# azuxmioy/Render-In-Between

Hardware: AMD Instinct MI355X
Metric: rendered frames/sec at 512x512 (generator forward + blend, device-resident) (higher is better)
Workload: dtype f32

## Files before the change

include/rib.h:

```cpp
#ifndef RIB_H
#define RIB_H

#include <stddef.h>
#include <stdint.h>

#ifdef __cplusplus
extern "C" {
#endif

typedef struct rib_handle rib_handle;

typedef enum {
  RIB_OK = 0,
  RIB_ERR_INVALID = -1,
  RIB_ERR_UNSUPPORTED = -2,
  RIB_ERR_STATE = -3,
  RIB_ERR_MISSING = -4,
  RIB_ERR_HIP = -5,
  RIB_ERR_WORKSPACE = -6
} rib_status;

typedef struct {
  int32_t label_nc;
  int32_t image_nc;
// ... 104 lines not shown
int rib_time_op(rib_handle* h, int B, int H, int W, const char* op_name, const float* label,
                const float* img_fake, const float* img_prev, float* img, float* mask, void* workspace,
                size_t workspace_bytes, int iters, void* hip_stream, double* usec);

int rib_set_graph_replay(rib_handle* h, int enable);
int rib_graph_stats(rib_handle* h, int64_t* captures, int64_t* replays);

int rib_set_plan_batch(rib_handle* h, int n);
int rib_get_plan_batch(const rib_handle* h);

const char* rib_build_info(void);

int rib_debug_conv_weight(rib_handle* h, const char* conv_name, float* w_oihw, float* bias);
int rib_debug_spade_weight(rib_handle* h, const char* conv_name, float* w_2c_by_cond, float* bias_2c);
int rib_debug_launch_info(rib_handle* h, int B, int H, int W, int idx, char* buf, size_t buflen);

#ifdef __cplusplus
}
#endif
#endif
```

render-in-between_amd/_native.py:

```python
from __future__ import annotations

import ctypes as C
import os

_HERE = os.path.dirname(os.path.abspath(__file__))
LIB_PATH = os.environ.get("RIB_LIBRARY") or os.path.join(_HERE, "csrc", "librib.so")

KC_NAMES = ("igemm", "spade", "stats", "pool", "eltwise", "pack", "conv_aux")


class RibConfig(C.Structure):
    _fields_ = [(n, C.c_int32) for n in (
        "label_nc", "image_nc", "num_filters", "max_num_filters", "num_layers", "num_down_img",
        "emb_filters", "emb_max_filters", "emb_down", "mask_filters", "mask_max_filters",
        "mask_down", "mask_res_blocks")]


class RibError(RuntimeError):
    def __init__(self, code, msg):
        super().__init__("rib error %d: %s" % (code, msg))
        self.code = code


_lib = None
# ... 47 lines not shown
    "rib_read_tap": (C.c_int, [C.c_void_p, C.c_int, C.c_int, C.c_int, C.c_int, C.c_void_p,
                               C.c_void_p, C.c_void_p]),
    "rib_profile_begin": (C.c_int, [C.c_void_p]),
    "rib_profile_begin_kernels": (C.c_int, [C.c_void_p]),
    "rib_profile_collect": (C.c_int, [C.c_void_p, C.POINTER(C.c_int64), C.POINTER(C.c_double)]),
    "rib_forward_flops": (C.c_int, [C.c_void_p, C.c_int, C.c_int, C.c_int, C.POINTER(C.c_double)]),
    "rib_num_launches": (C.c_int, [C.c_void_p, C.c_int, C.c_int, C.c_int]),
    "rib_num_variants": (C.c_int, []),
    "rib_variant_info": (C.c_int, [C.c_int, C.POINTER(C.c_int)]),
    "rib_set_choice": (C.c_int, [C.c_void_p, C.c_int, C.c_int, C.c_int, C.c_char_p, C.c_int, C.c_int]),
    "rib_time_op": (C.c_int, [C.c_void_p, C.c_int, C.c_int, C.c_int, C.c_char_p] + [C.c_void_p] * 6
                    + [C.c_size_t, C.c_int, C.c_void_p, C.POINTER(C.c_double)]),
    "rib_debug_conv_weight": (C.c_int, [C.c_void_p, C.c_char_p, C.c_void_p, C.c_void_p]),
    "rib_debug_spade_weight": (C.c_int, [C.c_void_p, C.c_char_p, C.c_void_p, C.c_void_p]),
    "rib_debug_launch_info": (C.c_int, [C.c_void_p, C.c_int, C.c_int, C.c_int, C.c_int, C.c_char_p, C.c_size_t]),
    "rib_build_info": (C.c_char_p, []),
    "rib_set_graph_replay": (C.c_int, [C.c_void_p, C.c_int]),
    "rib_graph_stats": (C.c_int, [C.c_void_p, C.POINTER(C.c_int64), C.POINTER(C.c_int64)]),
    "rib_set_plan_batch": (C.c_int, [C.c_void_p, C.c_int]),
    "rib_get_plan_batch": (C.c_int, [C.c_void_p]),
}


def lib():
    global _lib
    if _lib is None:
        if not os.path.exists(LIB_PATH):
            raise RuntimeError(
                "native library %s is missing: build it with "
                "`python render-in-between_amd/csrc/build.py` (there is no CPU fallback)" % LIB_PATH)
# ... 22 lines not shown
```

render-in-between_amd/csrc/kernels.hip.h:

```cpp
#pragma once
#include "igemm.hip.h"

namespace rib {

struct GemmDmaParams {
  const float* A; const float* B; float* C;
  int M, N, K, lda, ldc;
  size_t sA, sB, sC;
  int modB;
  int K2; unsigned long long kmask;
};

typedef uint32_t u32x4 __attribute__((ext_vector_type(4)));
__device__ __forceinline__ void split3_bf16(const float4 p, const float4 q, bf16x8& hi, bf16x8& mid, bf16x8& lo) {
  const float x[8] = {p.x, p.y, p.z, p.w, q.x, q.y, q.z, q.w};
  u32x4 h, m, l;
#pragma unroll
  for (int i = 0; i < 4; ++i) {
    const uint32_t u0 = __float_as_uint(x[2 * i]), u1 = __float_as_uint(x[2 * i + 1]);
    h[i] = __builtin_amdgcn_perm(u1, u0, 0x07060302u);
    const float r0 = x[2 * i] - __uint_as_float(u0 & 0xffff0000u), r1 = x[2 * i + 1] - __uint_as_float(u1 & 0xffff0000u);
    const uint32_t v0 = __float_as_uint(r0), v1 = __float_as_uint(r1);
    m[i] = __builtin_amdgcn_perm(v1, v0, 0x07060302u);
    const float s0 = r0 - __uint_as_float(v0 & 0xffff0000u), s1 = r1 - __uint_as_float(v1 & 0xffff0000u);
    l[i] = __builtin_amdgcn_perm(__float_as_uint(s1), __float_as_uint(s0), 0x07060302u);
  }
// ... 1 lines not shown
}

template <int WM, int WN, int NF, int ST = ST_F32, int X3 = 0>
__global__ __launch_bounds__(256) void k_gemm_dma(const GemmDmaParams p) {
  static_assert(WM * WN == 4, "4 waves per workgroup");
  static_assert(X3 == 0 || ST == ST_F32, "split products: fp32 storage");
  constexpr int BM = 32 * WM, BN = 32 * NF * WN, BK = 32;
  constexpr int EPW = ST == ST_F32 ? 1 : 2;
  constexpr int STAGE = (BM + BN) * BK;
  constexpr int NFILL = (BM + BN) / 32;
  __shared__ __attribute__((aligned(16))) float smem[2 * STAGE];
  const int tid = threadIdx.x, lane = tid & 63, li = lane & 31, lh = lane >> 5;
  const int wave = __builtin_amdgcn_readfirstlane(tid >> 6);
  const int wm = wave / WN, wn = wave % WN;
  const int m0 = blockIdx.x * BM, n0 = blockIdx.y * BN;
  const int z = blockIdx.z;
  const float* A = p.A + (size_t)z * p.sA / EPW;
  const float* B = p.B + (size_t)(p.modB ? z % p.modB : 0) * p.sB / EPW;
  f32x16 acc[NF];
  f32x16 acc_s[X3 == 2 ? NF : 1];
#pragma unroll
  for (int nf = 0; nf < NF; ++nf)
#pragma unroll
    for (int r = 0; r < 16; ++r) { acc[nf][r] = 0.f; if constexpr (X3 == 2) acc_s[nf][r] = 0.f; }
  const int ldb = (p.K + p.K2) / EPW;
  const int nch = (p.K + (p.K2 && ((p.kmask >> (z % p.modB)) & 1ull) ? p.K2 : 0)) / (BK * EPW);
  typedef __attribute__((address_space(3))) void lds_void;
  const uint32_t lds0 = (uint32_t)(size_t)(lds_void*)smem;
  const float* src[NFILL];
#pragma unroll
  for (int j = 0; j < NFILL; ++j) {
    const int trow = wave * 8 + 32 * j + (lane >> 3);
    const bool isA = 32 * j < BM;
    const int row = isA ? trow : trow - BM;
    const int ls = (lane & 7) ^ ((row >> 1) & 7);
    src[j] = isA ? A + (size_t)min(m0 + row, p.M - 1) * (p.lda / EPW) + ls * 4 : B + (size_t)min(n0 + row, p.N - 1) * ldb + ls * 4;
  }
  auto fill = [&](int st, int kc) {
#pragma unroll
    for (int j = 0; j < NFILL; ++j) {
      const uint32_t dst = lds0 + (uint32_t)(st * STAGE + (wave * 8 + 32 * j) * BK) * 4u;
// ... 46 lines not shown
#pragma unroll
      for (int nf = 0; nf < NF; ++nf) {
        if constexpr (ST == ST_F32) {
          acc[nf] = __builtin_amdgcn_mfma_f32_32x32x2f32(a.x, b[nf].x, acc[nf], 0, 0, 0);
          acc[nf] = __builtin_amdgcn_mfma_f32_32x32x2f32(a.y, b[nf].y, acc[nf], 0, 0, 0);
          acc[nf] = __builtin_amdgcn_mfma_f32_32x32x2f32(a.z, b[nf].z, acc[nf], 0, 0, 0);
          acc[nf] = __builtin_amdgcn_mfma_f32_32x32x2f32(a.w, b[nf].w, acc[nf], 0, 0, 0);
        } else if constexpr (ST == ST_F16) {
          acc[nf] = __builtin_amdgcn_mfma_f32_32x32x16_f16(*reinterpret_cast<const f16x8*>(&a), *reinterpret_cast<const f16x8*>(&b[nf]), acc[nf], 0, 0, 0);
        } else {
          acc[nf] = __builtin_amdgcn_mfma_f32_32x32x16_bf16(*reinterpret_cast<const bf16x8*>(&a), *reinterpret_cast<const bf16x8*>(&b[nf]), acc[nf], 0, 0, 0);
        }
      }
    }
  }
  float* C = p.C + (size_t)z * p.sC;
#pragma unroll
  for (int nf = 0; nf < NF; ++nf) {
    const int col = n0 + (wn * NF + nf) * 32 + li;
#pragma unroll
    for (int r = 0; r < 16; ++r) {
      const int row = m0 + wm * 32 + (r & 3) + 8 * (r >> 2) + 4 * lh;
      float v = acc[nf][r];
      if constexpr (X3 == 2) v += acc_s[nf][r];
      if (row < p.M && col < p.N) C[(size_t)row * p.ldc + col] = v;
    }
  }
}

struct FinalizeParams {
  const double* part;
// ... 340 lines not shown
  if constexpr (MODE2 >= 0) {
    const int n1 = p.nslices - p.nslices2;
    if (slice >= n1) { wino_in_slice<MODE2, true>(wino_second(p), slice - n1, ub, red, s_sc, s_sh); return; }
  }
  wino_in_slice<MODE, false>(p, slice, ub, red, s_sc, s_sh);
}

struct WinoOutParams {
  const float* m; int tilesY, tilesX, CoutPad;
  const float* bias;
  float* y; int yC, yoff, Cout, Hout, Wout;
  int act;
  const float* res; int resC;
  double* stat_part;
  int nslices, ublocks;
};

__device__ __forceinline__ void wino_out_partials(double (*red)[256][4], const double s1[4], const double s2[4], double* stat_part,
                                                  int n, int ublocks, int ub, int slice, int CoutPad) {
#pragma unroll
  for (int e = 0; e < 4; ++e) { red[0][threadIdx.x][e] = s1[e]; red[1][threadIdx.x][e] = s2[e]; }
  __syncthreads();
  if (threadIdx.x < 64) {
    const int c = slice * 64 + threadIdx.x;
    if (c < CoutPad) {
      const int g = threadIdx.x >> 2, e = threadIdx.x & 3;
      double a1 = 0.0, a2 = 0.0;
#pragma unroll
      for (int s = 0; s < 16; ++s) { a1 += red[0][s * 16 + g][e]; a2 += red[1][s * 16 + g][e]; }
      double* dst = stat_part + (((size_t)n * ublocks + ub) * 2) * CoutPad;
      dst[c] = a1;
      dst[CoutPad + c] = a2;
    }
  }
}

__global__ __launch_bounds__(256) void k_wino_out(const WinoOutParams p) {
  __shared__ __attribute__((aligned(16))) double red[2][256][4];
  const int c4n = p.CoutPad / 4;
  const int slice = blockIdx.x % p.nslices, ub = blockIdx.x / p.nslices;
  const int c4 = slice * 16 + (threadIdx.x & 15);
  const int n = blockIdx.y;
  const int ntiles = p.tilesY * p.tilesX;
  double s1[4] = {0.0, 0.0, 0.0, 0.0}, s2[4] = {0.0, 0.0, 0.0, 0.0};
  if (c4 < c4n) {
    const float4 bv = *reinterpret_cast<const float4*>(p.bias + c4 * 4);
    const size_t plane = (size_t)ntiles * p.CoutPad;
    for (int u = ub * 16 + (threadIdx.x >> 4); u < ntiles * 2; u += p.ublocks * 16) {
      const int r = u & 1, tile = u >> 1;
      const float* mb = p.m + (size_t)n * 16 * plane + (size_t)tile * p.CoutPad + c4 * 4;
      float4 mm[3][4];
#pragma unroll
      for (int a = 0; a < 3; ++a)
#pragma unroll
        for (int q = 0; q < 4; ++q) mm[a][q] = *reinterpret_cast<const float4*>(mb + (size_t)((r + a) * 4 + q) * plane);
      const float sg = r ? -1.f : 1.f;
      float4 uu[4];
#pragma unroll
      for (int q = 0; q < 4; ++q)
        uu[q] = make_float4(mm[0][q].x + sg * (mm[1][q].x + mm[2][q].x), mm[0][q].y + sg * (mm[1][q].y + mm[2][q].y),
                            mm[0][q].z + sg * (mm[1][q].z + mm[2][q].z), mm[0][q].w + sg * (mm[1][q].w + mm[2][q].w));
      float4 yv[2];
      yv[0] = RIB_F4_ADD(RIB_F4_ADD(uu[0], uu[1]), uu[2]);
      yv[1] = RIB_F4_SUB(RIB_F4_SUB(uu[1], uu[2]), uu[3]);
      const int ty = tile / p.tilesX, tx = tile % p.tilesX;
      const int oy = 2 * ty + r;
      float rr[2][4];
#pragma unroll
      for (int q = 0; q < 2; ++q) {
        const int cy = min(oy, p.Hout - 1), cx = min(2 * tx + q, p.Wout - 1);
// ... 112 lines not shown
  }
}

template <int MODE, int MODE2 = -1>
__global__ __launch_bounds__(256) void k_wino4_in(const WinoInParams p) {
  __shared__ double red[4 * 64 * 2];
  __shared__ float s_sc[64], s_sh[64];
  const int slice = blockIdx.x % p.nslices, ub = blockIdx.x / p.nslices;
  if constexpr (MODE2 >= 0) {
    const int n1 = p.nslices - p.nslices2;
    if (slice >= n1) { wino4_in_slice<MODE2, true>(wino_second(p), slice - n1, ub, red, s_sc, s_sh); return; }
  }
  wino4_in_slice<MODE, false>(p, slice, ub, red, s_sc, s_sh);
}

__global__ __launch_bounds__(256) void k_wino4_out(const WinoOutParams p) {
  __shared__ __attribute__((aligned(16))) double red[2][256][4];
  const int c4n = p.CoutPad / 4;
  const int slice = blockIdx.x % p.nslices, ub = blockIdx.x / p.nslices;
  const int c4 = slice * 16 + (threadIdx.x & 15);
  const int n = blockIdx.y;
  const int ntiles = p.tilesY * p.tilesX;
  double s1[4] = {0.0, 0.0, 0.0, 0.0}, s2[4] = {0.0, 0.0, 0.0, 0.0};
  if (c4 < c4n) {
    const float4 bv = *reinterpret_cast<const float4*>(p.bias + c4 * 4);
    const size_t plane = (size_t)ntiles * p.CoutPad;
    for (int unit = ub * 16 + (threadIdx.x >> 4); unit < ntiles * 4; unit += p.ublocks * 16) {
      const int tile = unit >> 2, r = unit & 3;
      const float* mb = p.m + (size_t)n * 36 * plane + (size_t)tile * p.CoutPad + c4 * 4;
      float4 u[6];
#pragma unroll
      for (int q = 0; q < 6; ++q) u[q] = make_float4(0.f, 0.f, 0.f, 0.f);
      const int ax = r == 0 ? 0 : 5;
      const float cx_ = (r == 0 || r == 3) ? 1.f : 0.f;
      float4 mm[5][6];
#pragma unroll
      for (int k = 0; k < 5; ++k)
#pragma unroll
        for (int q = 0; q < 6; ++q) mm[k][q] = *reinterpret_cast<const float4*>(mb + (size_t)((k < 4 ? k + 1 : ax) * 6 + q) * plane);
#pragma unroll
      for (int k = 0; k < 5; ++k) {
        const float coef = k < 4 ? kWino4AT[r][k + 1] : cx_;
#pragma unroll
        for (int q = 0; q < 6; ++q) u[q] = f4_fma(coef, mm[k][q], u[q]);
      }
      const float4 s12 = RIB_F4_ADD(u[1], u[2]);
      const float4 d12 = RIB_F4_SUB(u[1], u[2]);
      const float4 s34 = RIB_F4_ADD(u[3], u[4]);
      const float4 d34 = RIB_F4_SUB(u[3], u[4]);
      float4 yv[4];
      yv[0] = make_float4(u[0].x + s12.x + s34.x, u[0].y + s12.y + s34.y, u[0].z + s12.z + s34.z, u[0].w + s12.w + s34.w);
      yv[1] = f4_fma(3.f / 4, d12, f4_scale(3.f / 2, d34));
      yv[2] = f4_fma(9.f / 16, s12, f4_scale(9.f / 4, s34));
      yv[3] = f4_fma(27.f / 64, d12, f4_fma(27.f / 8, d34, u[5]));
// ... 653 lines not shown
```

render-in-between_amd/csrc/rib.hip:

```cpp
#include "kernels.hip.h"
#include "rib_host.h"
#include <hip/hip_ext.h>

#include <algorithm>
#include <array>
#include <climits>
#include <cmath>
#include <cstdio>
#include <cstdlib>
#include <cstring>
#include <map>
#include <memory>
#include <string>
#include <variant>
#include <vector>


#include "variants.hip.h"
#define RIB_V(sec, ...) RIB_I_V(RIB_F_EXTERN, __VA_ARGS__)
#define RIB_VK(sec, ...) RIB_I_VK(RIB_F_EXTERN, __VA_ARGS__)
#define RIB_VT(sec, ...) RIB_I_VT(RIB_F_EXTERN, __VA_ARGS__)
#define RIB_VTK(sec, ...) RIB_I_VTK(RIB_F_EXTERN, __VA_ARGS__)
#define RIB_V9(sec, ...) RIB_I_V9(RIB_F_EXTERN, __VA_ARGS__)
#define RIB_VU4(sec, ...) RIB_I_VU4(RIB_F_EXTERN, __VA_ARGS__)
// ... 786 lines not shown
struct FusionPolicy {
  bool consumer_stats = !getenv("RIB_NO_CONSUMER_STATS");
  bool head_conv = !getenv("RIB_NO_HEADCONV");
  bool small_conv = !getenv("RIB_NO_SMALLCONV");
  long wino_max_px = getenv("RIB_WINO_MAX_PX") ? atol(getenv("RIB_WINO_MAX_PX")) : 16384;
  int wino_force = getenv("RIB_WINO_M") ? atoi(getenv("RIB_WINO_M")) : 0;
  bool split_k = !getenv("RIB_NO_SPLITK");
  bool n16 = !getenv("RIB_NO_N16");
  int lowc_tw = getenv("RIB_LOWC_TW") ? (atoi(getenv("RIB_LOWC_TW")) == 16 ? 16 : 32) : 0;
  long cond_gemm_max_px = getenv("RIB_COND_GEMM_MAX_PX") ? atol(getenv("RIB_COND_GEMM_MAX_PX")) : 4096;
  bool unfused_spade = !getenv("RIB_NO_UNFUSED_SPADE");
  bool lazy_sources = !getenv("RIB_NO_LAZY");
  bool fuse_shortcut = !getenv("RIB_NO_FUSE_SHORTCUT");
  bool wino_shortcut = !getenv("RIB_NO_WINO_SHORTCUT");
  int wino_shortcut_m = getenv("RIB_WINO_SHORTCUT_M") ? atoi(getenv("RIB_WINO_SHORTCUT_M")) : 0;
  bool ws_reuse = !getenv("RIB_NO_WS_REUSE");
  static bool pair_mask_encoders() { return !getenv("RIB_NO_PAIR"); }
};

struct Builder {
  rib_handle* h;
  Plan* P;
  int B;
  const FusionPolicy pol;
  size_t ws = 0;
  std::string error;
  bool mark_label = false;
  bool pair_mask = false;
  bool defer_stats = true;
  void materialize(const Norm& n, const std::string& consumer = std::string()) {
// ... 107 lines not shown
  bool runs_wino(const ConvArgs& a, int Hout, int Wout, const std::string& opname = std::string()) const {
    const ConvDef& c = *a.cd;
    return h->prec() == PREC_F32 && (a.aux ? c.wino_s_ok : c.wino_ok) && !a.ups && !a.res_ups && !a.pair && !a.in.virt && a.y_nchw.sp == PS_NULL &&
           a.y_user.sp == PS_NULL && (long)Hout * Wout <= pol.wino_max_px && Hout >= 2 && Wout >= 2 &&
           (!a.aux || (!a.res && shortcut_wino_m(c, *a.aux, opname, Hout, Wout) != 0));
  }
  int default_wino_m(int Hout, int Wout) const { return (long)TB_() * ((Hout + 3) / 4) * ((Wout + 3) / 4) >= 256 ? 4 : 2; }
  int shortcut_wino_m(const ConvDef& c, const ConvDef& s, const std::string& opname, int Hout, int Wout) const {
    if (!pol.wino_shortcut || !pol.fuse_shortcut || opname.empty() || !c.fb_off || s.ks != 1 || s.coutp != c.coutp || s.cinp % 32 != 0 || c.cinp % 32 != 0) return 0;
    if (!pick_gemm_dma(h->prec(), 16, 64, c.coutp, c.cinp)) return 0;
    if (pol.wino_shortcut_m == 2 || pol.wino_shortcut_m == 4) return pol.wino_shortcut_m;
    const int d = default_wino_m(Hout, Wout);
    for (int m : {d, 6 - d})
      if (h->choices.count(fmt("%d,%d,%d|%s%s", TB_(), P->H, P->W, opname.c_str(), m == 2 ? ".wino" : ".wino4"))) return m;
    return 0;
  }
  bool would_wino(const ConvDef& cd, int H, int W) const { ConvArgs t; t.cd = &cd; return runs_wino(t, H, W); }

  bool conv(const ConvArgs& a, const std::string& opname) {
    const ConvDef& c = *a.cd;
    const int Hout = a.ups ? a.in.H * 2 : (c.stride == 2 ? a.in.H / 2 : a.in.H);
    const int Wout = a.ups ? a.in.W * 2 : (c.stride == 2 ? a.in.W / 2 : a.in.W);
    if (a.in.virt) return conv_lowc(a, opname);
    const int nB = a.pair ? 2 * B : B;
    if (a.pair) {
      const ConvDef& d = *a.pair;
      if (d.cinp != c.cinp || d.coutp != c.coutp || d.cout != c.cout || d.ks != c.ks || d.stride != c.stride || d.ups_in || c.ups_in || a.ups || a.res || a.aux ||
          a.y_nchw.sp != PS_NULL || a.y_user.sp != PS_NULL || a.y_none || !a.want_stats || c.in_affine != d.in_affine || d.w_off <= c.w_off || d.b_off <= c.b_off ||
          (c.in_affine && (d.g_off <= c.g_off || d.g_off - c.g_off != d.be_off - c.be_off)) || (h->mc16() && d.w16_off <= c.w16_off)) {
        error = opname + ": the two convolutions of a paired launch must have the same shape"; return false;
// ... 157 lines not shown
  }

  bool conv_wino(const ConvArgs& a, const std::string& opname, int Hout, int Wout) {
    const ConvDef& c = *a.cd;
    const int wino_force = pol.wino_force;
    const int wm = a.aux ? shortcut_wino_m(c, *a.aux, opname, Hout, Wout) : (wino_force == 2 || wino_force == 4 ? wino_force : default_wino_m(Hout, Wout));
    const int NP = (wm + 2) * (wm + 2);
    const int tilesY = (Hout + wm - 1) / wm, tilesX = (Wout + wm - 1) / wm, ntiles = tilesY * tilesX;
    const std::string gname = opname + (wm == 2 ? ".wino" : ".wino4");
    const int K2 = a.aux ? a.aux->cinp : 0, ldv = c.cinp + K2;
    unsigned long long kmask = 0;
    if (a.aux) {
      if (a.aux_in.Cp != K2 || a.aux_in.H != Hout || a.aux_in.W != Wout || a.in.H != Hout || a.in.W != Wout) { error = opname + ": fused shortcut operand does not fit"; return false; }
      for (int r = 1; r <= wm; ++r) for (int q = 1; q <= wm; ++q) kmask |= 1ull << (r * (wm + 2) + q);
    }
    const size_t v_off = alloc((size_t)B * NP * ntiles * ldv * sizeof(float));
    const size_t m_off = alloc((size_t)B * NP * ntiles * c.coutp * sizeof(float));
    {
      OpOf<WinoInParams> op(RIB_KC_CONVAUX, opname + ".wino_in"); op.for_op = gname; op.wino_m = wm;
      WinoInParams& wi = op.p();
      wi.H = a.in.H; wi.W = a.in.W; wi.xC = a.in.Cp; wi.Cin = c.cinp; wi.tilesY = tilesY; wi.tilesX = tilesX;
      wi.pro_lrelu = a.pro_lrelu ? 1 : 0; wi.ldv = ldv;
      op.bind(&WinoInParams::x, WS(a.in.off)); op.bind(&WinoInParams::v, WS(v_off));
      if (a.in.lazy) {
        const LazySrc& L = *a.in.lazy;
        if (a.pro || a.pro_lrelu) { error = gname + ": a lazy input carries its own prologue"; return false; }
        op.wi_mode = L.mode;
        op.bind(&WinoInParams::x, WS(L.x.off)); wi.xC = L.x.Cp;
        wi.pro_ld = L.nx.ld;
        if (!take_partials(L.nx, op, &WinoInParams::st)) { materialize(L.nx, gname); op.bind(&WinoInParams::pro_scale, WS(L.nx.sc)); op.bind(&WinoInParams::pro_shift, WS(L.nx.sh)); }
        if (L.mode == WSRC_SPADE) {
          wi.x_ups = L.x_ups ? 1 : 0; wi.pro_lrelu = L.lrelu ? 1 : 0;
// ... 24 lines not shown
          op.bind(&WinoInParams::slab2, WS(L.slab_off)); wi.slab2_ld = L.slab_ld; wi.col0_2 = L.col0; op.bind(&WinoInParams::sbias2, WT(L.sbias_off));
        } else op.bind(&WinoInParams::x2, WS(a.aux_in.off));
      }
      const int nsl = (c.cinp + 63) / 64 + wi.nslices2, units = ntiles * (wm + 2);
      wi.nslices = nsl; wi.ublocks = std::max(1, std::min((units + 15) / 16, (wi.st.tiles > 0 ? 512 : 4096) / nsl));
      op.grid = dim3(wi.ublocks * nsl, B, 1);
      push(op);
    }
    {
      Choice ch;
      ch.v = pick_gemm_dma(h->prec(), (long)TB_() * NP, ntiles, c.coutp, c.cinp);
      if (!ch.v) ch = choose_variant(h->prec(), 1, 1, false, false, c.coutp, TB_() * NP, tilesY, tilesX, c.cinp, false, 0, false);
      auto it = h->choices.find(fmt("%d,%d,%d|%s", TB_(), P->H, P->W, gname.c_str()));
      if (it != h->choices.end()) {
        const Variant& tv = kVariants[it->second.first];
        if (tv.BF16 != h->prec() || tv.KS != 1 || tv.STRIDE != 1 || tv.UPS || tv.SPADE || tv.NF == 0 || c.cinp % tv.BK != 0 || it->second.second != 1 || (a.aux && !tv.dma())) {
          error = fmt("%s: tuned choice (variant %d, ksplit %d) does not fit this layer", gname.c_str(), it->second.first, it->second.second); return false;
        }
        ch.v = &tv; ch.ksplit = 1;
      }
      const Variant* v = ch.v;
      if (!v) { error = gname + ": no 1x1 kernel variant"; return false; }
      if (a.aux && !v->dma()) { error = gname + ": the fused shortcut needs a k_gemm_dma tile"; return false; }
      const int set = ensure_wino_set(h, (int)(&c - h->convs.data()), wm, a.aux ? (int)(a.aux - h->convs.data()) : -1);
      if (set < 0) { error = gname + ": " + h->err; return false; }
      const double fl = 2.0 * c.cin * 9.0 * c.cout * (double)Hout * Wout * B + (a.aux ? 2.0 * a.aux->cin * a.aux->cout * (double)Hout * Wout * B : 0.0);
      P->flops[RIB_KC_IGEMM] += fl;
      if (v->dma()) {
        OpOf<GemmDmaParams> op(RIB_KC_IGEMM, gname); op.var = v; op.wino = true; op.wino_m = wm; op.flops = fl;
        GemmDmaParams& g = op.p();
        g.M = ntiles; g.N = c.coutp; g.K = c.cinp; g.lda = ldv; g.ldc = c.coutp;
        g.sA = (size_t)ntiles * ldv; g.sB = (size_t)c.coutp * ldv; g.sC = (size_t)ntiles * c.coutp; g.modB = NP;
        g.K2 = K2; g.kmask = kmask;
        op.bind(&GemmDmaParams::A, WS(v_off)); op.bind(&GemmDmaParams::B, WINO(set)); op.bind(&GemmDmaParams::C, WS(m_off));
        op.grid = dim3((ntiles + v->BM() - 1) / v->BM(), (c.coutp + v->BN() - 1) / v->BN(), B * NP);
        push(op);
      } else {
      OpOf<IgemmParams> op(RIB_KC_IGEMM, gname); op.var = v; op.wino = true; op.wino_m = wm; op.flops = fl;
      IgemmParams& p = op.p();
      p.Hin = tilesY; p.Win = tilesX; p.xC = c.cinp; p.Cin = c.cinp; p.CoutPad = c.coutp; p.Hout = tilesY; p.Wout = tilesX;
      p.tilesX = (tilesX + v->TW() - 1) / v->TW(); p.tilesY = (tilesY + v->TH() - 1) / v->TH(); p.xcd_chunk = xcd_chunk_of(p.tilesX * p.tilesY);
      p.act = ACT_NONE; p.ksplit = 1; p.yC = c.coutp; p.yoff = 0; p.Cout = c.coutp;
      p.w_mod = NP; p.w_stride = (unsigned)((size_t)c.coutp * c.cinp);
      op.bind(&IgemmParams::x, WS(v_off)); op.bind(&IgemmParams::w, WINO(set)); op.bind(&IgemmParams::bias, WT(c.zero_off)); op.bind(&IgemmParams::y, WS(m_off));
      op.grid = dim3(p.tilesX * p.tilesY, (c.coutp + v->BN() - 1) / v->BN(), B * NP);
      push(op);
      }
    }
    {
      OpOf<WinoOutParams> op(RIB_KC_CONVAUX, opname + ".wino_out"); op.for_op = gname; op.wino_m = wm;
      WinoOutParams& wo = op.p();
      const int nsl = (c.coutp + 63) / 64, units = ntiles * wm;
      const int blocks = std::max(1, std::min((units + 15) / 16, (int)STATS_MAX_PARTIALS));
      wo.tilesY = tilesY; wo.tilesX = tilesX; wo.CoutPad = c.coutp; wo.ublocks = blocks; wo.nslices = nsl;
      wo.yC = a.out.Cp; wo.yoff = a.yoff; wo.Cout = a.cout_store >= 0 ? a.cout_store : h->padc(c.cout);
      wo.Hout = Hout; wo.Wout = Wout; wo.act = a.act;
      if (a.out.H != Hout || a.out.W != Wout) { error = fmt("%s: output size mismatch", opname.c_str()); return false; }
      op.bind(&WinoOutParams::m, WS(m_off)); op.bind(&WinoOutParams::bias, WT(a.aux ? c.fb_off : c.b_off)); op.bind(&WinoOutParams::y, WS(a.out.off));
      if (a.res) { op.bind(&WinoOutParams::res, WS(a.res->off)); wo.resC = a.res->Cp; }
      size_t part_off = 0;
      if (a.want_stats) { part_off = alloc((size_t)B * blocks * 2 * c.coutp * sizeof(double)); op.bind(&WinoOutParams::stat_part, WS(part_off)); }
      op.grid = dim3(blocks * nsl, B, 1);
      push(op);
      if (a.want_stats) {
        OpOf<FinalizeParams> f = finalize_op(opname, part_off, blocks, c.coutp, h->padc(c.cout), *a.stats_out, a.stats_choff, Hout, Wout, a.affine ? &c : nullptr, B);
        finalize_or_defer(f, a.stats_out, a.stats_choff != 0 || a.stats_now, part_off, blocks, c.coutp, f.p().inv_count, a.affine, c.g_off, c.be_off);
      }
    }
    return true;
  }

// ... 735 lines not shown
          else if (s1) RIB_KLAUNCH((K<WSRC_SPADE, WSRC_PLAIN>), op.grid, dim3(256), 0, st, p);              \
          else if (s2) RIB_KLAUNCH((K<WSRC_PLAIN, WSRC_SPADE>), op.grid, dim3(256), 0, st, p);              \
          else RIB_KLAUNCH((K<WSRC_PLAIN, WSRC_PLAIN>), op.grid, dim3(256), 0, st, p)
          if (op.wino_m == 4) { RIB_WINO_IN2(k_wino4_in); } else { RIB_WINO_IN2(k_wino_in); }
#undef RIB_WINO_IN2
        } else if (op.wino_m == 4) {
          if (op.wi_mode == WSRC_SPADE) RIB_KLAUNCH(k_wino4_in<WSRC_SPADE>, op.grid, dim3(256), 0, st, p);
          else if (op.wi_mode == WSRC_JOIN) RIB_KLAUNCH(k_wino4_in<WSRC_JOIN>, op.grid, dim3(256), 0, st, p);
          else RIB_KLAUNCH(k_wino4_in<WSRC_PLAIN>, op.grid, dim3(256), 0, st, p);
        } else {
          if (op.wi_mode == WSRC_SPADE) RIB_KLAUNCH(k_wino_in<WSRC_SPADE>, op.grid, dim3(256), 0, st, p);
          else if (op.wi_mode == WSRC_JOIN) RIB_KLAUNCH(k_wino_in<WSRC_JOIN>, op.grid, dim3(256), 0, st, p);
          else RIB_KLAUNCH(k_wino_in<WSRC_PLAIN>, op.grid, dim3(256), 0, st, p);
        }
      } break;
      case OP_WINO_OUT:
        if (op.wino_m == 4) RIB_KLAUNCH(k_wino4_out, op.grid, dim3(256), 0, st, std::get<WinoOutParams>(params));
        else RIB_KLAUNCH(k_wino_out, op.grid, dim3(256), 0, st, std::get<WinoOutParams>(params));
        break;
      case OP_LOWC: launch_lowc(op.lowc_ce, op.lowc_ncol, op.lowc_tw, op.grid, st, std::get<LowcParams>(params)); break;
      case OP_PACK: RIB_LAUNCH_ST(bf16, k_pack, op.grid, dim3(256), 0, st, std::get<PackParams>(params)); break;
    }
  }
  g_prof_pair = ProfPair();
  if (h->profiling && !h->prof_kernels) {
    hipEvent_t e1 = nullptr;
    HIP_TRY(h, hipEventCreate(&e1));
    HIP_TRY(h, hipEventRecord(e1, st));
    h->prof_events.push_back({-1, e1});
  }
  HIP_TRY(h, hipGetLastError());
  return RIB_OK;
}

// ... 566 lines not shown
    bias_2c[sg.C + ch] = h->host_blob[sg.b_off + colb];
  }
  return RIB_OK;
}

static int launch_info_head(const Op& op, char* buf, size_t buflen) {
  if (op.kind() == OP_IGEMM && op.small_co > 0)
    snprintf(buf, buflen, "%s|%d|%u,%u,%u|%s 16x16 tile, %d output channels%s|%.0f", op.name.c_str(), op.kclass, op.grid.x, op.grid.y, op.grid.z,
             op.head ? "head (taps as MFMA columns)" : "direct (vector ALUs)", op.small_co, op.fuse_blend ? " + fused blend" : "", op.flops);
  else if (op.kind() == OP_IGEMM)
    snprintf(buf, buflen, "%s|%d|%u,%u,%u|tile %dx%d BN %d BK %d s%d k%d ups%d ksplit%d kw%d tb%d%s v%d|%.0f", op.name.c_str(), op.kclass, op.grid.x, op.grid.y, op.grid.z,
             op.var->TH(), op.var->TW(), op.var->BN(), op.var->BK, op.var->STRIDE, op.var->KS, (int)op.var->UPS, op.as<IgemmParams>().ksplit, op.var->KW, op.var->DMAK ? 100 + (op.var->TB == 9 ? 9 : 0) : op.var->TB,
             op.wino ? (op.wino_m == 4 ? " wino4" : " wino") : "", (int)(op.var - kVariants), op.flops);
  else if (op.kind() == OP_GEMM)
    snprintf(buf, buflen, "%s|%d|%u,%u,%u|gemm (LDS-DMA staged operands) tile %dx%d BK 32, %d x [%d x %d x %d]%s|%.0f", op.name.c_str(), op.kclass, op.grid.x, op.grid.y, op.grid.z,
             op.var->BM(), op.var->BN(), (int)op.grid.z, op.as<GemmDmaParams>().M, op.as<GemmDmaParams>().N, op.as<GemmDmaParams>().K, (std::string(op.wino ? (op.wino_m == 4 ? " wino4" : " wino") : "") + (op.as<GemmDmaParams>().K2 ? fmt(" + K %d of the 1x1 shortcut at %d positions", op.as<GemmDmaParams>().K2, __builtin_popcountll(op.as<GemmDmaParams>().kmask)) : std::string())).c_str(), op.flops);
  else if (op.kind() == OP_LOWC)
    snprintf(buf, buflen, "%s|%d|%u,%u,%u|lowc (caller's NCHW tensors, K = 9 x %d real channels) 8x%d tile, %d columns|%.0f", op.name.c_str(), op.kclass,
             op.grid.x, op.grid.y, op.grid.z, op.lowc_ce, op.lowc_tw, op.lowc_ncol, op.flops);
  else
    snprintf(buf, buflen, "%s|%d|%u,%u,%u||0", op.name.c_str(), op.kclass, op.grid.x, op.grid.y, op.grid.z);
  return RIB_OK;
}

static double op_algorithmic_bytes(const rib_handle* h, const Plan* P, const Op& op) {
  const double e = h->esz(), Bn = P->B;
  switch (op.kind()) {
    case OP_IGEMM: {
      const IgemmParams& p = op.as<IgemmParams>();
      const double samples = p.pair ? 2.0 * Bn : Bn;
      const int taps = op.var ? op.var->KS * op.var->KS : 9;
// ... 3 lines not shown
      if (op.var && op.var->SPADE) {
        b += Bn * p.Hout * p.Wout * (double)p.C * e / (p.xm_ups ? 4.0 : 1.0);
        b += Bn * p.Hout * p.Wout * (double)p.C * e * p.nsets;
      } else if (op.bound(&IgemmParams::slab)) {
        b += (double)p.ksplit * samples * p.Hout * p.Wout * p.CoutPad * 4.0;
      } else {
        b += samples * p.Hout * p.Wout * (double)p.Cout * (op.small_co > 0 || p.y_f32 ? 4.0 : e);
        if (op.bound(&IgemmParams::res)) b += samples * p.Hout * p.Wout * (double)p.Cout * e / (p.res_ups ? 4.0 : 1.0);
        if (op.bound(&IgemmParams::x2)) b += samples * p.Hout * p.Wout * (double)p.Cin2 * e + (double)p.CoutPad * p.Cin2 * e;
        if (op.fuse_blend) b += Bn * p.Hout * p.Wout * 3.0 * 4.0 * 3.0;
      }
      return b;
    }
    case OP_GEMM: {
      const GemmDmaParams& g = op.as<GemmDmaParams>();
      const double Z = op.grid.z;
      const double z2 = g.K2 ? Bn * __builtin_popcountll(g.kmask) : 0.0, nb2 = g.K2 ? (double)__builtin_popcountll(g.kmask) : 0.0;
      return Z * g.M * (double)g.K * e + (g.modB ? (double)g.modB : 1.0) * g.N * (double)g.K * e + Z * g.M * (double)g.N * 4.0 +
             z2 * g.M * (double)g.K2 * e + nb2 * g.N * (double)g.K2 * e;
    }
    case OP_LOWC: {
      const LowcParams& l = op.as<LowcParams>();
      return Bn * l.H * l.W * (double)(l.c0 + l.c1 + l.c2) * 4.0 + Bn * l.H * l.W * (double)l.Cout * e + 9.0 * (l.c0 + l.c1 + l.c2) * l.Cout * 4.0;
    }
    case OP_POOL: { const PoolParams& q = op.as<PoolParams>(); return Bn * q.H * q.W * (double)q.C * e * 1.25; }
    case OP_INADD: { const InAddParams& q = op.as<InAddParams>(); return Bn * q.HW * (double)q.C * e * 3.0; }
    case OP_SPLITEPI: {
      const SplitEpiParams& q = op.as<SplitEpiParams>();
      return (double)q.ksplit * q.B * q.Hout * q.Wout * q.CoutPad * 4.0 + (double)q.B * q.Hout * q.Wout * q.Cout * e * (op.bound(&SplitEpiParams::res) ? 2.0 : 1.0);
    }
    case OP_MODULATE: {
      const ModulateParams& m = op.as<ModulateParams>();
      const double px = (double)m.B * m.Hout * m.Wout;
// ... 2 lines not shown
    case OP_WINO_IN: {
      const WinoInParams& w = op.as<WinoInParams>();
      const int T = op.wino_m + 2;
      double b = Bn * w.H * w.W * (double)w.Cin * e / (w.x_ups ? 4.0 : 1.0) + Bn * w.tilesY * w.tilesX * (double)T * T * w.Cin * e;
      if (op.wi_mode != 0 && op.bound(&WinoInParams::slab)) b += Bn * w.H * w.W * 2.0 * w.Cin * 4.0;
      if (op.wi_mode2 >= 0) {
        b += Bn * w.H * w.W * (double)w.Cin2 * e / (w.x2_ups ? 4.0 : 1.0) + Bn * w.tilesY * w.tilesX * (double)op.wino_m * op.wino_m * w.Cin2 * e;
        if (op.bound(&WinoInParams::slab2)) b += Bn * w.H * w.W * 2.0 * w.Cin2 * 4.0;
      } else
      if (op.bound(&WinoInParams::x2) || op.bound(&WinoInParams::xres)) b += Bn * w.H * w.W * (double)w.Cin * e * 2.0;
      return b;
    }
    case OP_WINO_OUT: {
      const WinoOutParams& w = op.as<WinoOutParams>();
      const int T = op.wino_m + 2;
      return Bn * w.tilesY * w.tilesX * (double)T * T * w.CoutPad * 4.0 + Bn * w.Hout * w.Wout * (double)w.Cout * e * (op.bound(&WinoOutParams::res) ? 2.0 : 1.0);
    }
    case OP_FINALIZE: { const FinalizeParams& q = op.as<FinalizeParams>(); return Bn * q.tiles * 2.0 * q.Cs * 8.0; }
    default: return 0.0;
  }
}

int rib_debug_launch_info(rib_handle* h, int B, int H, int W, int idx, char* buf, size_t buflen) {
  if (!h || !buf) return RIB_ERR_INVALID;
  Plan* P = get_plan(h, B, H, W);
  if (!P || idx < 0 || idx >= (int)P->ops.size()) return RIB_ERR_INVALID;
  const Op& op = P->ops[idx];
  const int rc = launch_info_head(op, buf, buflen);
  const size_t n = strlen(buf);
  if (n + 24 < buflen) snprintf(buf + n, buflen - n, "|%.0f", op_algorithmic_bytes(h, P, op));
  return rc;
}

const char* rib_build_info(void) {
  static const std::string info = [] {
#define RIB_X(s) rib_stamp_section_##s,
    const char* sh[RIB_NSECTIONS] = {RIB_FOR_SECTIONS(RIB_X)};
#undef RIB_X
    std::string s = std::string("librib stamp=") + (kLibStamp + sizeof("rib-stamp lib ") - 1) + " shards=";
    bool ok = true;
    for (int i = 0; i < RIB_NSECTIONS; ++i) {
      const char* hash = strrchr(sh[i], ' ');
      hash = hash ? hash + 1 : "?";
      ok = ok && strcmp(hash, RIB_SHARD_STAMP) == 0;
      s += std::string(i ? "," : "") + hash;
    }
// ... 133 lines not shown
```

Baseline: 399.4.

## Split fused shortcut K into separate GEMM slices summed in winograd output

In Winograd convolutions that fuse a 1x1 shortcut, the interior positions carry extra K2 channels and take longer than the other batch planes, which unbalances the batched GEMM. This change moves the shortcut channels into their own z-slices (K2 split into nsplit pieces) that write extra partial planes. The Winograd output kernel (new XP template) then adds those planes back before its transform. It costs extra workspace and extra output-plane reads, in exchange for more parallel, evenly sized GEMM blocks.

```diff
diff --git a/include/rib.h b/include/rib.h
--- a/include/rib.h
+++ b/include/rib.h
@@ -142,6 +142,7 @@
 int rib_debug_conv_weight(rib_handle* h, const char* conv_name, float* w_oihw, float* bias);
 int rib_debug_spade_weight(rib_handle* h, const char* conv_name, float* w_2c_by_cond, float* bias_2c);
 int rib_debug_launch_info(rib_handle* h, int B, int H, int W, int idx, char* buf, size_t buflen);
+int rib_debug_gemm_slice(int modB, int K, int K2, unsigned long long kmask, int nmain, int nsplit, int bz, int out[5]);
 
 #ifdef __cplusplus
 }
diff --git a/render-in-between_amd/_native.py b/render-in-between_amd/_native.py
--- a/render-in-between_amd/_native.py
+++ b/render-in-between_amd/_native.py
@@ -85,6 +85,7 @@
     "rib_debug_conv_weight": (C.c_int, [C.c_void_p, C.c_char_p, C.c_void_p, C.c_void_p]),
     "rib_debug_spade_weight": (C.c_int, [C.c_void_p, C.c_char_p, C.c_void_p, C.c_void_p]),
     "rib_debug_launch_info": (C.c_int, [C.c_void_p, C.c_int, C.c_int, C.c_int, C.c_int, C.c_char_p, C.c_size_t]),
+    "rib_debug_gemm_slice": (C.c_int, [C.c_int, C.c_int, C.c_int, C.c_ulonglong, C.c_int, C.c_int, C.c_int, C.POINTER(C.c_int)]),
     "rib_build_info": (C.c_char_p, []),
     "rib_set_graph_replay": (C.c_int, [C.c_void_p, C.c_int]),
     "rib_graph_stats": (C.c_int, [C.c_void_p, C.POINTER(C.c_int64), C.POINTER(C.c_int64)]),
diff --git a/render-in-between_amd/csrc/kernels.hip.h b/render-in-between_amd/csrc/kernels.hip.h
--- a/render-in-between_amd/csrc/kernels.hip.h
+++ b/render-in-between_amd/csrc/kernels.hip.h
@@ -9,7 +9,29 @@
   size_t sA, sB, sC;
   int modB;
   int K2; unsigned long long kmask;
+  int nmain, nsplit;
 };
+
+struct GemmDmaSlice { int zA, pos, k0, klen, zC; };
+__host__ __device__ __forceinline__ GemmDmaSlice gemm_dma_slice(int modB, int K, int K2, unsigned long long kmask, int nmain, int nsplit, int bz) {
+  GemmDmaSlice s;
+  if (nsplit > 0) {
+    const int nmark = __builtin_popcountll(kmask), nx = nmain / modB * nmark * nsplit;
+    if (bz < nx) {
+      const int piece = bz % nsplit, j = bz / nsplit % nmark, n = bz / (nsplit * nmark);
+      unsigned long long m = kmask;
+      for (int i = 0; i < j; ++i) m &= m - 1;
+      s.pos = __builtin_ctzll(m);
+      s.zA = n * modB + s.pos; s.zC = nmain + bz;
+      s.klen = K2 / nsplit; s.k0 = K + piece * s.klen;
+      return s;
+    }
+    bz -= nx;
+  }
+  s.zA = s.zC = bz; s.pos = modB ? bz % modB : 0; s.k0 = 0;
+  s.klen = K + (nsplit == 0 && K2 && ((kmask >> s.pos) & 1ull) ? K2 : 0);
+  return s;
+}
 
 typedef uint32_t u32x4 __attribute__((ext_vector_type(4)));
 __device__ __forceinline__ void split3_bf16(const float4 p, const float4 q, bf16x8& hi, bf16x8& mid, bf16x8& lo) {
@@ -41,9 +63,9 @@
   const int wave = __builtin_amdgcn_readfirstlane(tid >> 6);
   const int wm = wave / WN, wn = wave % WN;
   const int m0 = blockIdx.x * BM, n0 = blockIdx.y * BN;
-  const int z = blockIdx.z;
-  const float* A = p.A + (size_t)z * p.sA / EPW;
-  const float* B = p.B + (size_t)(p.modB ? z % p.modB : 0) * p.sB / EPW;
+  const GemmDmaSlice sl = gemm_dma_slice(p.modB, p.K, p.K2, p.kmask, p.nmain, p.nsplit, blockIdx.z);
+  const float* A = p.A + ((size_t)sl.zA * p.sA + sl.k0) / EPW;
+  const float* B = p.B + ((size_t)sl.pos * p.sB + sl.k0) / EPW;
   f32x16 acc[NF];
   f32x16 acc_s[X3 == 2 ? NF : 1];
 #pragma unroll
@@ -51,7 +73,7 @@
 #pragma unroll
     for (int r = 0; r < 16; ++r) { acc[nf][r] = 0.f; if constexpr (X3 == 2) acc_s[nf][r] = 0.f; }
   const int ldb = (p.K + p.K2) / EPW;
-  const int nch = (p.K + (p.K2 && ((p.kmask >> (z % p.modB)) & 1ull) ? p.K2 : 0)) / (BK * EPW);
+  const int nch = sl.klen / (BK * EPW);
   typedef __attribute__((address_space(3))) void lds_void;
   const uint32_t lds0 = (uint32_t)(size_t)(lds_void*)smem;
   const float* src[NFILL];
@@ -128,7 +150,7 @@
       }
     }
   }
-  float* C = p.C + (size_t)z * p.sC;
+  float* C = p.C + (size_t)sl.zC * p.sC;
 #pragma unroll
   for (int nf = 0; nf < NF; ++nf) {
     const int col = n0 + (wn * NF + nf) * 32 + li;
@@ -499,6 +521,7 @@
   const float* res; int resC;
   double* stat_part;
   int nslices, ublocks;
+  int xplanes, xbase; unsigned long long xmask;
 };
 
 __device__ __forceinline__ void wino_out_partials(double (*red)[256][4], const double s1[4], const double s2[4], double* stat_part,
@@ -520,6 +543,7 @@
   }
 }
 
+template <bool XP>
 __global__ __launch_bounds__(256) void k_wino_out(const WinoOutParams p) {
   __shared__ __attribute__((aligned(16))) double red[2][256][4];
   const int c4n = p.CoutPad / 4;
@@ -539,6 +563,23 @@
       for (int a = 0; a < 3; ++a)
 #pragma unroll
         for (int q = 0; q < 4; ++q) mm[a][q] = *reinterpret_cast<const float4*>(mb + (size_t)((r + a) * 4 + q) * plane);
+      if constexpr (XP) {
+        const float* xb = p.m + ((size_t)p.xbase + (size_t)n * 4 * p.xplanes) * plane + (size_t)tile * p.CoutPad + c4 * 4;
+        for (int s = 0; s < p.xplanes; ++s) {
+          float4 x[2][2];
+#pragma unroll
+          for (int i = 0; i < 2; ++i)
+#pragma unroll
+            for (int j = 0; j < 2; ++j) x[i][j] = *reinterpret_cast<const float4*>(xb + (size_t)((i * 2 + j) * p.xplanes + s) * plane);
+#pragma unroll
+          for (int i = 0; i < 2; ++i)
+#pragma unroll
+            for (int j = 0; j < 2; ++j) {
+              const float4 lo = RIB_F4_ADD(mm[i][1 + j], x[i][j]), hi = RIB_F4_ADD(mm[1 + i][1 + j], x[i][j]);
+              if (r) mm[i][1 + j] = lo; else mm[1 + i][1 + j] = hi;
+            }
+        }
+      }
       const float sg = r ? -1.f : 1.f;
       float4 uu[4];
 #pragma unroll
@@ -681,6 +722,7 @@
   wino4_in_slice<MODE, false>(p, slice, ub, red, s_sc, s_sh);
 }
 
+template <bool XP>
 __global__ __launch_bounds__(256) void k_wino4_out(const WinoOutParams p) {
   __shared__ __attribute__((aligned(16))) double red[2][256][4];
   const int c4n = p.CoutPad / 4;
@@ -705,6 +747,18 @@
       for (int k = 0; k < 5; ++k)
 #pragma unroll
         for (int q = 0; q < 6; ++q) mm[k][q] = *reinterpret_cast<const float4*>(mb + (size_t)((k < 4 ? k + 1 : ax) * 6 + q) * plane);
+      if constexpr (XP) {
+        const float* xb = p.m + ((size_t)p.xbase + (size_t)n * 16 * p.xplanes) * plane + (size_t)tile * p.CoutPad + c4 * 4;
+        for (int s = 0; s < p.xplanes; ++s) {
+#pragma unroll
+          for (int k = 0; k < 4; ++k)
+#pragma unroll
+            for (int j = 0; j < 4; ++j) {
+              const float4 x = *reinterpret_cast<const float4*>(xb + (size_t)((k * 4 + j) * p.xplanes + s) * plane);
+              mm[k][1 + j] = RIB_F4_ADD(mm[k][1 + j], x);
+            }
+        }
+      }
 #pragma unroll
       for (int k = 0; k < 5; ++k) {
         const float coef = k < 4 ? kWino4AT[r][k + 1] : cx_;
diff --git a/render-in-between_amd/csrc/rib.hip b/render-in-between_amd/csrc/rib.hip
--- a/render-in-between_amd/csrc/rib.hip
+++ b/render-in-between_amd/csrc/rib.hip
@@ -824,6 +824,8 @@
   bool fuse_shortcut = !getenv("RIB_NO_FUSE_SHORTCUT");
   bool wino_shortcut = !getenv("RIB_NO_WINO_SHORTCUT");
   int wino_shortcut_m = getenv("RIB_WINO_SHORTCUT_M") ? atoi(getenv("RIB_WINO_SHORTCUT_M")) : 0;
+  bool wino_kslices = !getenv("RIB_NO_WINO_KSLICES");
+  int wino_kslices_force = getenv("RIB_WINO_KSLICES") ? atoi(getenv("RIB_WINO_KSLICES")) : -1;
   bool ws_reuse = !getenv("RIB_NO_WS_REUSE");
   static bool pair_mask_encoders() { return !getenv("RIB_NO_PAIR"); }
 };
@@ -961,6 +963,16 @@
     for (int m : {d, 6 - d})
       if (h->choices.count(fmt("%d,%d,%d|%s%s", TB_(), P->H, P->W, opname.c_str(), m == 2 ? ".wino" : ".wino4"))) return m;
     return 0;
+  }
+  int shortcut_kslices(int K, int K2, const std::string& gname) const {
+    if (!pol.wino_kslices || K2 <= 0) return 0;
+    auto fits = [&](int n) { return n >= 1 && K2 % (32 * n) == 0; };
+    int rule = 1;
+    while (!(fits(rule) && K2 / rule <= K)) ++rule;
+    if (pol.wino_kslices_force >= 0) return fits(pol.wino_kslices_force) ? pol.wino_kslices_force : rule;
+    auto it = h->choices.find(fmt("%d,%d,%d|%s", TB_(), P->H, P->W, gname.c_str()));
+    if (it != h->choices.end()) return it->second.second - 1;
+    return rule;
   }
   bool would_wino(const ConvDef& cd, int H, int W) const { ConvArgs t; t.cd = &cd; return runs_wino(t, H, W); }
 
@@ -1148,8 +1160,11 @@
       if (a.aux_in.Cp != K2 || a.aux_in.H != Hout || a.aux_in.W != Wout || a.in.H != Hout || a.in.W != Wout) { error = opname + ": fused shortcut operand does not fit"; return false; }
       for (int r = 1; r <= wm; ++r) for (int q = 1; q <= wm; ++q) kmask |= 1ull << (r * (wm + 2) + q);
     }
+    const int nsplit = a.aux ? shortcut_kslices(c.cinp, K2, gname) : 0;
+    const int nmark = __builtin_popcountll(kmask);
+    if (a.aux && (nsplit < 0 || (nsplit > 0 && K2 % (32 * nsplit) != 0))) { error = fmt("%s: tuned choice asks for %d K slices of the shortcut's %d channels", gname.c_str(), nsplit, K2); return false; }
     const size_t v_off = alloc((size_t)B * NP * ntiles * ldv * sizeof(float));
-    const size_t m_off = alloc((size_t)B * NP * ntiles * c.coutp * sizeof(float));
+    const size_t m_off = alloc((size_t)B * (NP + nmark * nsplit) * ntiles * c.coutp * sizeof(float));
     {
       OpOf<WinoInParams> op(RIB_KC_CONVAUX, opname + ".wino_in"); op.for_op = gname; op.wino_m = wm;
       WinoInParams& wi = op.p();
@@ -1204,7 +1219,7 @@
       auto it = h->choices.find(fmt("%d,%d,%d|%s", TB_(), P->H, P->W, gname.c_str()));
       if (it != h->choices.end()) {
         const Variant& tv = kVariants[it->second.first];
-        if (tv.BF16 != h->prec() || tv.KS != 1 || tv.STRIDE != 1 || tv.UPS || tv.SPADE || tv.NF == 0 || c.cinp % tv.BK != 0 || it->second.second != 1 || (a.aux && !tv.dma())) {
+        if (tv.BF16 != h->prec() || tv.KS != 1 || tv.STRIDE != 1 || tv.UPS || tv.SPADE || tv.NF == 0 || c.cinp % tv.BK != 0 || (it->second.second != 1 && !a.aux) || (a.aux && !tv.dma())) {
           error = fmt("%s: tuned choice (variant %d, ksplit %d) does not fit this layer", gname.c_str(), it->second.first, it->second.second); return false;
         }
         ch.v = &tv; ch.ksplit = 1;
@@ -1221,9 +1236,9 @@
         GemmDmaParams& g = op.p();
         g.M = ntiles; g.N = c.coutp; g.K = c.cinp; g.lda = ldv; g.ldc = c.coutp;
         g.sA = (size_t)ntiles * ldv; g.sB = (size_t)c.coutp * ldv; g.sC = (size_t)ntiles * c.coutp; g.modB = NP;
-        g.K2 = K2; g.kmask = kmask;
+        g.K2 = K2; g.kmask = kmask; g.nmain = B * NP; g.nsplit = nsplit;
         op.bind(&GemmDmaParams::A, WS(v_off)); op.bind(&GemmDmaParams::B, WINO(set)); op.bind(&GemmDmaParams::C, WS(m_off));
-        op.grid = dim3((ntiles + v->BM() - 1) / v->BM(), (c.coutp + v->BN() - 1) / v->BN(), B * NP);
+        op.grid = dim3((ntiles + v->BM() - 1) / v->BM(), (c.coutp + v->BN() - 1) / v->BN(), B * (NP + nmark * nsplit));
         push(op);
       } else {
       OpOf<IgemmParams> op(RIB_KC_IGEMM, gname); op.var = v; op.wino = true; op.wino_m = wm; op.flops = fl;
@@ -1245,6 +1260,7 @@
       wo.tilesY = tilesY; wo.tilesX = tilesX; wo.CoutPad = c.coutp; wo.ublocks = blocks; wo.nslices = nsl;
       wo.yC = a.out.Cp; wo.yoff = a.yoff; wo.Cout = a.cout_store >= 0 ? a.cout_store : h->padc(c.cout);
       wo.Hout = Hout; wo.Wout = Wout; wo.act = a.act;
+      wo.xplanes = nsplit; wo.xmask = nsplit ? kmask : 0ull; wo.xbase = B * NP;
       if (a.out.H != Hout || a.out.W != Wout) { error = fmt("%s: output size mismatch", opname.c_str()); return false; }
       op.bind(&WinoOutParams::m, WS(m_off)); op.bind(&WinoOutParams::bias, WT(a.aux ? c.fb_off : c.b_off)); op.bind(&WinoOutParams::y, WS(a.out.off));
       if (a.res) { op.bind(&WinoOutParams::res, WS(a.res->off)); wo.resC = a.res->Cp; }
@@ -2010,10 +2026,11 @@
           else RIB_KLAUNCH(k_wino_in<WSRC_PLAIN>, op.grid, dim3(256), 0, st, p);
         }
       } break;
-      case OP_WINO_OUT:
-        if (op.wino_m == 4) RIB_KLAUNCH(k_wino4_out, op.grid, dim3(256), 0, st, std::get<WinoOutParams>(params));
-        else RIB_KLAUNCH(k_wino_out, op.grid, dim3(256), 0, st, std::get<WinoOutParams>(params));
-        break;
+      case OP_WINO_OUT: {
+        const bool xp = std::get<WinoOutParams>(params).xplanes > 0;
+        if (op.wino_m == 4) { if (xp) RIB_KLAUNCH(k_wino4_out<true>, op.grid, dim3(256), 0, st, std::get<WinoOutParams>(params)); else RIB_KLAUNCH(k_wino4_out<false>, op.grid, dim3(256), 0, st, std::get<WinoOutParams>(params)); }
+        else { if (xp) RIB_KLAUNCH(k_wino_out<true>, op.grid, dim3(256), 0, st, std::get<WinoOutParams>(params)); else RIB_KLAUNCH(k_wino_out<false>, op.grid, dim3(256), 0, st, std::get<WinoOutParams>(params)); }
+      } break;
       case OP_LOWC: launch_lowc(op.lowc_ce, op.lowc_ncol, op.lowc_tw, op.grid, st, std::get<LowcParams>(params)); break;
       case OP_PACK: RIB_LAUNCH_ST(bf16, k_pack, op.grid, dim3(256), 0, st, std::get<PackParams>(params)); break;
     }
@@ -2610,7 +2627,8 @@
              op.wino ? (op.wino_m == 4 ? " wino4" : " wino") : "", (int)(op.var - kVariants), op.flops);
   else if (op.kind() == OP_GEMM)
     snprintf(buf, buflen, "%s|%d|%u,%u,%u|gemm (LDS-DMA staged operands) tile %dx%d BK 32, %d x [%d x %d x %d]%s|%.0f", op.name.c_str(), op.kclass, op.grid.x, op.grid.y, op.grid.z,
-             op.var->BM(), op.var->BN(), (int)op.grid.z, op.as<GemmDmaParams>().M, op.as<GemmDmaParams>().N, op.as<GemmDmaParams>().K, (std::string(op.wino ? (op.wino_m == 4 ? " wino4" : " wino") : "") + (op.as<GemmDmaParams>().K2 ? fmt(" + K %d of the 1x1 shortcut at %d positions", op.as<GemmDmaParams>().K2, __builtin_popcountll(op.as<GemmDmaParams>().kmask)) : std::string())).c_str(), op.flops);
+             op.var->BM(), op.var->BN(), (int)op.grid.z, op.as<GemmDmaParams>().M, op.as<GemmDmaParams>().N, op.as<GemmDmaParams>().K, (std::string(op.wino ? (op.wino_m == 4 ? " wino4" : " wino") : "") + (op.as<GemmDmaParams>().K2 ? fmt(" + K %d of the 1x1 shortcut at %d positions", op.as<GemmDmaParams>().K2, __builtin_popcountll(op.as<GemmDmaParams>().kmask)) : std::string()) +
+              (op.as<GemmDmaParams>().nsplit ? fmt(", as %d K slices of their own each", op.as<GemmDmaParams>().nsplit) : std::string())).c_str(), op.flops);
   else if (op.kind() == OP_LOWC)
     snprintf(buf, buflen, "%s|%d|%u,%u,%u|lowc (caller's NCHW tensors, K = 9 x %d real channels) 8x%d tile, %d columns|%.0f", op.name.c_str(), op.kclass,
              op.grid.x, op.grid.y, op.grid.z, op.lowc_ce, op.lowc_tw, op.lowc_ncol, op.flops);
@@ -2644,9 +2662,9 @@
     }
     case OP_GEMM: {
       const GemmDmaParams& g = op.as<GemmDmaParams>();
-      const double Z = op.grid.z;
+      const double Zc = op.grid.z, Z = g.nsplit ? (double)g.nmain : Zc;
       const double z2 = g.K2 ? Bn * __builtin_popcountll(g.kmask) : 0.0, nb2 = g.K2 ? (double)__builtin_popcountll(g.kmask) : 0.0;
-      return Z * g.M * (double)g.K * e + (g.modB ? (double)g.modB : 1.0) * g.N * (double)g.K * e + Z * g.M * (double)g.N * 4.0 +
+      return Z * g.M * (double)g.K * e + (g.modB ? (double)g.modB : 1.0) * g.N * (double)g.K * e + Zc * g.M * (double)g.N * 4.0 +
              z2 * g.M * (double)g.K2 * e + nb2 * g.N * (double)g.K2 * e;
     }
     case OP_LOWC: {
@@ -2679,7 +2697,8 @@
     case OP_WINO_OUT: {
       const WinoOutParams& w = op.as<WinoOutParams>();
       const int T = op.wino_m + 2;
-      return Bn * w.tilesY * w.tilesX * (double)T * T * w.CoutPad * 4.0 + Bn * w.Hout * w.Wout * (double)w.Cout * e * (op.bound(&WinoOutParams::res) ? 2.0 : 1.0);
+      const double planes = (double)T * T + (double)__builtin_popcountll(w.xmask) * w.xplanes;
+      return Bn * w.tilesY * w.tilesX * planes * w.CoutPad * 4.0 + Bn * w.Hout * w.Wout * (double)w.Cout * e * (op.bound(&WinoOutParams::res) ? 2.0 : 1.0);
     }
     case OP_FINALIZE: { const FinalizeParams& q = op.as<FinalizeParams>(); return Bn * q.tiles * 2.0 * q.Cs * 8.0; }
     default: return 0.0;
@@ -2695,6 +2714,15 @@
   const size_t n = strlen(buf);
   if (n + 24 < buflen) snprintf(buf + n, buflen - n, "|%.0f", op_algorithmic_bytes(h, P, op));
   return rc;
+}
+
+int rib_debug_gemm_slice(int modB, int K, int K2, unsigned long long kmask, int nmain, int nsplit, int bz, int out[5]) {
+  const int nmark = __builtin_popcountll(kmask);
+  if (!out || modB <= 0 || modB > 64 || nmain <= 0 || nmain % modB != 0 || nsplit < 0 || (nsplit > 0 && (nmark == 0 || K2 % nsplit != 0)) ||
+      (modB < 64 && (kmask >> modB)) || bz < 0 || bz >= nmain + nmain / modB * nmark * nsplit) return RIB_ERR_INVALID;
+  const GemmDmaSlice s = gemm_dma_slice(modB, K, K2, kmask, nmain, nsplit, bz);
+  out[0] = s.zA; out[1] = s.pos; out[2] = s.k0; out[3] = s.klen; out[4] = s.zC;
+  return RIB_OK;
 }
 
 const char* rib_build_info(void) {
```

Result: no change. 399.2 (-0.0%).
